# kcroker/Gadget-2.0.7-ngravs

Hardware: AMD Instinct MI355X
Metric: particle-steps/s (tree+PM) (higher is better)
Workload: dtype f64

## Files before the change

### gadget-2.0.7-ngravs_amd/__init__.py

```python
import ctypes as C
import os
import subprocess

import numpy as np

from . import abi, ic
from .abi import (Config, Particles, Stats, make_config, WALK_GROUP, WALK_STRICT,
                  LAW_NONE, LAW_NEWTON, LAW_NEG_NEWTON, LAW_YUKAWA, LAW_COLOYUK, LAW_BAMBAM, LAW_SOURCEBAM, LAW_TARGETBAM)

_HERE = os.path.dirname(os.path.abspath(__file__))
LIB_PATH = os.path.join(_HERE, "libngravs_hip.so")
_LIB = None

EXPORTS = [
    "ngravs_abi_version", "ngravs_build_info", "ngravs_config_default", "ngravs_create", "ngravs_destroy",
    "ngravs_set_fatal_handler", "ngravs_set_opening", "ngravs_set_walk_mode", "ngravs_set_softening", "ngravs_dd_record_bytes", "ngravs_get_config", "ngravs_set_tuning",
    "ngravs_memcpy", "ngravs_device_alloc", "ngravs_device_free",
    "ngravs_set_particles",
    "ngravs_set_old_acc", "ngravs_update_particles", "ngravs_force_update_tree", "ngravs_domain_decomposition", "ngravs_discard_grav_pm",
    "ngravs_force_treebuild", "ngravs_gravity_tree",
    "ngravs_pmforce_periodic", "ngravs_compute_accelerations", "ngravs_get_accel", "ngravs_get_stats", "ngravs_walk_unopened",
    "ngravs_get_domain", "ngravs_get_keys", "ngravs_get_order", "ngravs_get_shard", "ngravs_last_error",
    "ngravs_peano_hilbert_key", "ngravs_peano_keys", "ngravs_shortrange_table", "ngravs_direct_sum", "ngravs_direct_sum_targets",
    "ngravs_dd_num_local", "ngravs_dd_local_extent", "ngravs_dd_set_extent", "ngravs_get_domain_extent", "ngravs_dd_set_toptree",
    "ngravs_dd_get_toptree", "ngravs_dd_peano_order", "ngravs_dd_leaf_sums", "ngravs_dd_target_bounds", "ngravs_dd_keep_margin", "ngravs_dd_pack", "ngravs_dd_get_dest",
    "ngravs_dd_pack_leaves", "ngravs_dd_set_top", "ngravs_dd_recv_buffer", "ngravs_dd_apply_migration", "ngravs_dd_set_halo",
    "ngravs_dd_leaf_sums_kept", "ngravs_dd_pack_leaves_kept", "ngravs_dd_refresh_halo", "ngravs_dd_update_top", "ngravs_dd_get_kept",
    "ngravs_dd_set_ids", "ngravs_dd_get_ids",
    "ngravs_pm_slab_begin", "ngravs_pm_slab_pack", "ngravs_pm_slab_unpack", "ngravs_pm_slab_bytes",
]
HOST_EXPORTS = ["ngravs_host_comm_selftest", "ngravs_host_kept_step", "ngravs_host_toptree_borrow", "ngravs_host_domain_decomposition", "ngravs_host_domain_owners", "ngravs_host_domain_halo",
                "ngravs_host_plan_free", "ngravs_host_pmforce_periodic", "ngravs_host_compute_accelerations", "ngravs_host_split",
                "ngravs_host_pm_seconds", "ngravs_host_toptree_init", "ngravs_host_toptree_from_children", "ngravs_host_toptree_adapt",
                "ngravs_host_toptree_free", "ngravs_host_import_request", "ngravs_host_import_request_margin"]
RCCL_LIB_PATH = os.path.join(_HERE, "libngravs_rccl.so")
RCCL_EXPORTS = ["ngravs_rccl_selftest", "ngravs_rccl_unique_id", "ngravs_rccl_create", "ngravs_rccl_fill", "ngravs_rccl_destroy", "ngravs_rccl_stats",
                "ngravs_rccl_last_error", "ngravs_rccl_world", "ngravs_rccl_barrier", "ngravs_rccl_set_timeout"]


# ... 16 lines not shown
            raise NgravsError("libngravs_hip.so is not built (run __graft_entry__.build()); there is no CPU fallback")
        L = C.CDLL(LIB_PATH)
        L.ngravs_build_info.restype = C.c_char_p
        L.ngravs_last_error.restype = C.c_char_p
        L.ngravs_last_error.argtypes = [C.c_void_p]
        L.ngravs_peano_hilbert_key.restype = C.c_int64
        L.ngravs_peano_hilbert_key.argtypes = [C.c_int] * 4
        L.ngravs_force_treebuild.restype = C.c_int64
        L.ngravs_force_treebuild.argtypes = [C.c_void_p]
        for name in ("ngravs_destroy", "ngravs_domain_decomposition", "ngravs_gravity_tree",
                     "ngravs_pmforce_periodic", "ngravs_discard_grav_pm"):
            getattr(L, name).argtypes = [C.c_void_p]
        L.ngravs_compute_accelerations.argtypes = [C.c_void_p, C.c_int]
        L.ngravs_set_opening.argtypes = [C.c_void_p, C.c_double, C.c_double]
        L.ngravs_set_walk_mode.argtypes = [C.c_void_p, C.c_int]
        L.ngravs_set_softening.argtypes = [C.c_void_p, C.c_void_p]
        L.ngravs_dd_record_bytes.restype = C.c_int64
        L.ngravs_dd_record_bytes.argtypes = [C.c_void_p, C.c_int]
        L.ngravs_set_particles.argtypes = [C.c_void_p, C.c_void_p]
        L.ngravs_set_old_acc.argtypes = [C.c_void_p, C.c_void_p, C.c_int64, C.c_int]
        L.ngravs_get_accel.argtypes = [C.c_void_p, C.c_void_p, C.c_int64, C.c_void_p, C.c_int64, C.c_void_p, C.c_int64,
                                       C.c_void_p, C.c_int64, C.c_int, C.c_int]
        L.ngravs_set_tuning.argtypes = [C.c_void_p, C.c_char_p, C.c_double]
        L.ngravs_memcpy.argtypes = [C.c_void_p, C.c_void_p, C.c_void_p, C.c_int64, C.c_int]
        L.ngravs_get_stats.argtypes = [C.c_void_p, C.c_void_p]
        L.ngravs_get_domain.argtypes = [C.c_void_p, C.c_void_p]
        L.ngravs_get_keys.argtypes = [C.c_void_p, C.c_void_p, C.c_int]
        L.ngravs_get_order.argtypes = [C.c_void_p, C.c_void_p, C.c_int]
        L.ngravs_get_shard.argtypes = [C.c_void_p, C.c_void_p, C.c_void_p]
        L.ngravs_peano_keys.argtypes = [C.c_void_p, C.c_void_p, C.c_int64, C.c_void_p, C.c_double, C.c_int, C.c_void_p]
        L.ngravs_shortrange_table.argtypes = [C.c_void_p, C.c_void_p, C.c_void_p]
        L.ngravs_direct_sum.argtypes = [C.c_void_p, C.c_void_p, C.c_int64, C.c_void_p]
        L.ngravs_direct_sum_targets.argtypes = [C.c_void_p, C.c_void_p, C.c_void_p, C.c_void_p, C.c_int64, C.c_void_p]
        L.ngravs_dd_local_extent.argtypes = [C.c_void_p, C.c_void_p, C.c_void_p]
        L.ngravs_dd_set_extent.argtypes = [C.c_void_p, C.c_void_p, C.c_void_p]
        L.ngravs_get_config.argtypes = [C.c_void_p, C.c_void_p]
        L.ngravs_host_split.argtypes = [C.c_void_p, C.c_void_p, C.c_int64, C.c_int, C.c_double, C.c_void_p]
        L.ngravs_dd_pack.argtypes = [C.c_void_p, C.c_int, C.c_void_p, C.c_int, C.c_int, C.c_void_p, C.c_void_p, C.c_void_p]
        L.ngravs_host_toptree_init.argtypes = [C.c_void_p, C.c_int]
        L.ngravs_host_toptree_from_children.argtypes = [C.c_void_p, C.c_void_p, C.c_int32]
        L.ngravs_host_toptree_adapt.argtypes = [C.c_void_p, C.c_void_p, C.c_double, C.c_int, C.c_void_p]
        L.ngravs_host_toptree_free.argtypes = [C.c_void_p]
        L.ngravs_host_toptree_free.restype = None
        L.ngravs_host_import_request.argtypes = [C.c_void_p, C.c_void_p, C.c_void_p, C.c_void_p, C.c_void_p, C.c_int, C.c_void_p, C.c_void_p]
        L.ngravs_dd_apply_migration.argtypes = [C.c_void_p, C.c_void_p, C.c_int64]
        L.ngravs_dd_set_halo.argtypes = [C.c_void_p, C.c_void_p, C.c_int64]
# ... 241 lines not shown
```

### gadget-2.0.7-ngravs_amd/csrc/capi.hip

```cpp
#include "engine.hpp"
#include "../../include/ngravs_peano.h"
#include <chrono>
#include <cmath>

void ngravs_report(ngravs_ctx *ctx, int code, const std::string &msg)
{
  if(ctx)
    ctx->last_error = msg;
  if(ctx && ctx->on_fatal)
    ctx->on_fatal(code, msg.c_str());
  else
    fprintf(stderr, "task %d: endrun called with an error level of %d (%s)\n", ctx ? ctx->cfg.rank : 0, code, msg.c_str());
}

__global__ void k_pack_strided_f64(const unsigned char *src, long long stride, int ncomp, long long n, double *dst)
{
  long long i = blockIdx.x * (long long)blockDim.x + threadIdx.x;
  if(i >= n)
    return;
  const double *s = reinterpret_cast<const double *>(src + i * stride);
  for(int k = 0; k < ncomp; k++)
    dst[i * ncomp + k] = s[k];
}
__global__ void k_pack_type(const unsigned char *src, long long stride, long long n, int *dst, int *nbad)
// ... 409 lines not shown
    }
  else if(k == "walk_root")
    t.walk_root = iv != 0;
  else if(k == "walk_compact")
    t.walk_compact = iv != 0;
  else if(k == "walk_spread" && iv >= 0 && iv <= 64 && (iv & (iv - 1)) == 0)
    t.walk_spread = (int)iv;
  else if(k == "walk_sg" && iv >= 0 && iv <= 16)
    t.walk_sg = (int)iv;
  else if(k == "walk_ring" && iv >= 0 && iv <= 1)
    t.walk_ring = (int)iv;
  else if(k == "walk_ring_k" && iv >= 0 && iv <= 8)
    t.walk_ring_k = (int)iv;
  else if(k == "walk_nleaf" && iv >= -1 && iv <= 8)
    t.walk_nleaf = (int)iv;
  else if(k == "walk_exact_reach")
    t.walk_exact_reach = iv != 0;
  else if(k == "pm_notile")
    t.pm_notile = iv != 0;
  else if(k == "pm_fused_gather")
    t.pm_fused_gather = iv != 0;
  else if(k == "pm_tile_gather")
    t.pm_tile_gather = iv != 0;
  else if(k == "sort_full")
    t.sort_full = iv != 0;
  else if(k == "pm_tile8")
    t.pm_tile8 = iv != 0;
  else if(k == "tree_levelwise")
    t.tree_levelwise = iv != 0;
  else if(k == "dd_keep" && v >= 0 && v <= 0.25)
    t.dd_keep = v;
  else if(k == "moments_octet")
    t.moments_octet = iv != 0;
  else
    {
      ngravs_report(c, NGRAVS_ERR_ARG, "ngravs_set_tuning: unknown name or value out of range: " + k);
      return NGRAVS_ERR_ARG;
    }
  return NGRAVS_OK;
}

extern "C" int ngravs_memcpy(ngravs_ctx *c, void *dst, const void *src, int64_t bytes, int kind)
{
  if(!c || bytes < 0 || kind < 1 || kind > 3 || (bytes > 0 && (!dst || !src)))
    return NGRAVS_ERR_ARG;
  if(bytes == 0)
    return NGRAVS_OK;
  (void)hipSetDevice(c->cfg.device);
  HIP_TRY(c, hipStreamSynchronize(c->stream));
  HIP_TRY(c, hipMemcpy(dst, src, (size_t)bytes, kind == 1 ? hipMemcpyHostToDevice : (kind == 2 ? hipMemcpyDeviceToHost : hipMemcpyDeviceToDevice)));
  return NGRAVS_OK;
}

extern "C" int ngravs_device_alloc(ngravs_ctx *c, void **ptr, int64_t bytes)
{
  if(!c || !ptr || bytes < 0)
    return NGRAVS_ERR_ARG;
  *ptr = nullptr;
  (void)hipSetDevice(c->cfg.device);
  if(hipMalloc(ptr, (size_t)(bytes > 0 ? bytes : 1)) != hipSuccess)
    return NGRAVS_ERR_NOMEM;
// ... 1061 lines not shown
```

### gadget-2.0.7-ngravs_amd/csrc/engine.hpp

```cpp
#pragma once
#include <hip/hip_runtime.h>
#include <cstdint>
#include <cstdio>
#include <cstdlib>
#include <cstring>
#include <string>
#include <vector>
#include "../../include/ngravs_host.h"

#define NG_MAX NGRAVS_MAX_GRAVS
#define NTAB NGRAVS_NTAB
#define TREE_BITS NGRAVS_TREE_BITS
#define FLAG_BUCKET 64
#define FLAG_PSEUDO 128
#define FLAG_PARTIAL 256
#define MAX_LEVELS (TREE_BITS + 1)

struct ngravs_ctx;

#define HIP_TRY(ctx, expr)                                                                        \
  do                                                                                              \
    {                                                                                             \
      hipError_t e__ = (expr);                                                                    \
      if(e__ != hipSuccess)                                                                       \
// ... 57 lines not shown
  double ec[4];
  int src_in_box;
  int bam;
  int law_accel[NG_MAX][NG_MAX], law_spline[NG_MAX][NG_MAX];

};

struct TreeView
{
  const int *first, *count, *child, *flags;
  const int *npart;
  const double4 *geo, *mom;
  int nnodes;
  const int *ltab;
  int ltab_level;
  double ltab_corner[3], ltab_cl;
};

struct Tuning
{
  int walk_fused = 0, walk_waves = 0, walk_lcap = 0, walk_root = 0, walk_compact = 1, walk_spread = 0, walk_exact_reach = 0, walk_sg = 0, walk_nleaf = -1;
  long long walk_batch = 0;
  int pm_notile = 0, pm_fused_gather = 0, pm_tile_gather = 0, pm_tile8 = 0;
  int sort_full = 0;
  int tree_levelwise = 0;
  int moments_octet = 0;
  double dd_keep = 0;
  int walk_ring = 1;
  int walk_ring_k = 0;
};

#define TOP_CW(ng) (7 + 4 * (ng))
struct TopTree
{
  double total_count = 0;
  bool on = false;
  double import_reach = 0;
  ngravs_toptree h = {0, 0, 0, 0, nullptr, nullptr, nullptr, nullptr, nullptr};
  DevBuf<int> child, leaf;
  DevBuf<int> gcnt;
  DevBuf<unsigned char> info;
  DevBuf<double> gsum;
  DevBuf<int> leaf_owner;
  DevBuf<unsigned long long> reqmask;
  DevBuf<double> leaf_sums;
  DevBuf<int> own_leaf;
// ... 84 lines not shown
  DevBuf<int> d_levels;
  long long level_hint[MAX_LEVELS + 2] = {0};
  DevBuf<double> table;
  bool table_ready = false;
  DevBuf<double> lat;
  bool lat_ready = false;
  DevBuf<int> walk_stack;
  DevBuf<int> walk_tlist;
  DevBuf<unsigned char> walk_tmp;
  long long walk_ntargets = -1;
  bool walk_dense_tlist = false;
  int walk_spread = 0;
  int walk_sg = 1;
  long long walk_unopened = 0;
  int walk_unit_state = 4;
  double walk_ia_ratio = 0;
  bool all_active = true;
  DevBuf<int> walk_ovf;
  DevBuf<int> walk_counters;
  DevBuf<double> r_acc, r_pm, r_oldacc;
  DevBuf<int> r_nint;
  int pm_plan_n = 0;
  void *fft_fwd = nullptr, *fft_inv = nullptr;
  DevBuf<double> pm_rho;
  DevBuf<double> pm_force;
  DevBuf<double> pm_phi;
  DevBuf<double> pm_orig;
  DevBuf<double> out_tmp;
  DevBuf<float> out_tmpf;
  std::vector<unsigned char> host_stage;
  ngravs_stats_t stats;
  hipEvent_t ev0 = nullptr, ev1 = nullptr, evk0 = nullptr, evk1 = nullptr;
  std::vector<hipEvent_t> ev_batch;
  int walk_batches = 0;
  int walk_lcap = 0;
  int walk_scap = 0;
  std::string last_error;
};

int dom_find_extent(ngravs_ctx *c);
int dom_keys_and_sort(ngravs_ctx *c);
int dom_keys_only(ngravs_ctx *c, const double *d_pos, int64_t n, const double corner[3], double fac, int bits,
                  long long *d_keys);
int dd_local_extent(ngravs_ctx *c, double lo[3], double hi[3]);
void dd_apply_extent(ngravs_ctx *c, const double lo[3], const double hi[3]);
int dd_set_toptree(ngravs_ctx *c, int nnode, const int *child);
// ... 17 lines not shown
int tree_top_leaf_len(ngravs_ctx *c, double *dev_kept_sums, int stride);
int tree_top_refit(ngravs_ctx *c);
int dom_regather(ngravs_ctx *c);
static inline bool cfg_has_bam(const ngravs_config_t &cfg)
{
  for(int i = 0; i < cfg.n_gravs; i++)
    for(int j = 0; j < cfg.n_gravs; j++)
      if(cfg.law_accel[i][j] >= NGRAVS_LAW_BAMBAM || cfg.law_spline[i][j] >= NGRAVS_SPLINE_BAMBAM)
        return true;
  return false;
}
void make_walk_params(const ngravs_ctx *c, WalkParams *wp);
int walk_run(ngravs_ctx *c);
int walk_finish(ngravs_ctx *c);
int direct_run(ngravs_ctx *c, const int *d_idx, int64_t nt, double *d_acc);
int direct_run_targets(ngravs_ctx *c, const double4 *d_tpm, const int *d_ttype, int64_t nt, double *d_acc);
int eval_ring_slots(const WalkParams &wp, bool yuk, int waves);
int launch_eval_ring(ngravs_ctx *c, const TreeView &tv, const WalkParams &wp, bool yuk, int nblk, int waves, int K, const int *region,
                     const int *gcount, long long g0, long long nb, int lcap, int scap, int S, const int *tlist, int SG, long long t_count);
int pm_run(ngravs_ctx *c);
int pm_deposit(ngravs_ctx *c);
int pm_finish(ngravs_ctx *c);
void pm_release(ngravs_ctx *c);
int pmslab_begin(ngravs_ctx *c, int rank, int world, int bbox[6]);
int pmslab_pack(ngravs_ctx *c, int stage, const int *all_bbox, int64_t *send_counts, int64_t *recv_counts, void **send, void **recv);
int pmslab_unpack(ngravs_ctx *c, int stage);
void pmslab_release(ngravs_ctx *c);
void host_shortrange_table(const ngravs_config_t *cfg, double *force, double *pot);
double cfg_asmth(const ngravs_config_t *c);
double cfg_rcut(const ngravs_config_t *c);
```

### gadget-2.0.7-ngravs_amd/csrc/kernels_pm.hip

```cpp
#include "engine.hpp"
#include "pm_common.hpp"
#include <hipfft/hipfft.h>

__global__ void k_cic_deposit(const double4 *__restrict__ s_pm, const unsigned char *__restrict__ s_type,
                              const unsigned char *__restrict__ s_flag, long long n,
                              double to_slab, int N, int ng, const int *__restrict__ t2g_tab, double *__restrict__ rho)
{
  long long i = blockIdx.x * (long long)blockDim.x + threadIdx.x;
  if(i >= n || (s_flag[i] & 2))
    return;
  double4 p = s_pm[i];
  int g = t2g_tab[s_type[i]];
  const long long NZ = N + 2;
  double *grid = rho + (size_t)g * N * N * NZ;
  double dx, dy, dz;
  int sx = cell_of(p.x, to_slab, N, &dx), sy = cell_of(p.y, to_slab, N, &dy), sz = cell_of(p.z, to_slab, N, &dz);
  int sxx = sx + 1 == N ? 0 : sx + 1, syy = sy + 1 == N ? 0 : sy + 1, szz = sz + 1 == N ? 0 : sz + 1;
  double m = p.w;
  atomicAdd(&grid[((long long)sx * N + sy) * NZ + sz], m * (1.0 - dx) * (1.0 - dy) * (1.0 - dz));
  atomicAdd(&grid[((long long)sx * N + syy) * NZ + sz], m * (1.0 - dx) * dy * (1.0 - dz));
  atomicAdd(&grid[((long long)sx * N + sy) * NZ + szz], m * (1.0 - dx) * (1.0 - dy) * dz);
  atomicAdd(&grid[((long long)sx * N + syy) * NZ + szz], m * (1.0 - dx) * dy * dz);
  atomicAdd(&grid[((long long)sxx * N + sy) * NZ + sz], m * (dx) * (1.0 - dy) * (1.0 - dz));
  atomicAdd(&grid[((long long)sxx * N + syy) * NZ + sz], m * (dx)*dy * (1.0 - dz));
  atomicAdd(&grid[((long long)sxx * N + sy) * NZ + szz], m * (dx) * (1.0 - dy) * dz);
  atomicAdd(&grid[((long long)sxx * N + syy) * NZ + szz], m * (dx)*dy * dz);
}

template <int NG>
__global__ void k_green(const double2 *__restrict__ rho, double2 *__restrict__ phi, GreenParams gp)
{
  const int N = gp.N, NH = N / 2 + 1;
  long long idx = blockIdx.x * (long long)blockDim.x + threadIdx.x;
  long long total = (long long)N * N * NH;
  if(idx >= total)
    return;
  int z = (int)(idx % NH);
  int y = (int)((idx / NH) % N);
  int x = (int)(idx / ((long long)NH * N));
  double2 out[NG];
  green_mode<NG>(gp, x, y, z, rho, (size_t)total, (size_t)idx, out);
#pragma unroll
  for(int b = 0; b < NG; b++)
    phi[(size_t)b * total + idx] = out[b];
}

__global__ void k_gradient_gather(const double4 *__restrict__ s_pm, const unsigned char *__restrict__ s_type,
                                  const unsigned char *__restrict__ s_flag,
                                  long long first, long long n, double to_slab, int N, const int *__restrict__ t2g_tab,
                                  const double *__restrict__ phi, double fac, double *__restrict__ r_pm)
{
  long long i = blockIdx.x * (long long)blockDim.x + threadIdx.x;
  if(i >= n)
    return;
  i += first;
  if(s_flag[i] & 2)
    {
      r_pm[3 * i + 0] = r_pm[3 * i + 1] = r_pm[3 * i + 2] = 0.0;
      return;
    }
  double4 p = s_pm[i];
  int g = t2g_tab[s_type[i]];
  const long long NZ = N + 2;
  const double *grid = phi + (size_t)g * N * N * NZ;
  double dx, dy, dz;
  int sx = cell_of(p.x, to_slab, N, &dx), sy = cell_of(p.y, to_slab, N, &dy), sz = cell_of(p.z, to_slab, N, &dz);
  double wx[2] = {1.0 - dx, dx}, wy[2] = {1.0 - dy, dy}, wz[2] = {1.0 - dz, dz};
// ... 366 lines not shown
  r_pm[3 * i + 1] = acc[1];
  r_pm[3 * i + 2] = acc[2];
}

static int pm_tile_level(const ngravs_ctx *c, double to_slab, double max_cells = 16.0)
{
  if(!c->have_tree || c->tune.pm_notile)
    return -1;
  double len = c->dom[6];
  for(int l = 0; l < c->nlevels && l < TREE_BITS; l++, len *= 0.5)
    if(len * to_slab <= max_cells * 1.002)
      return (c->level_start[l + 1] - c->level_start[l] > 0) ? l : -1;
  return -1;
}

void pm_release(ngravs_ctx *c)
{
  if(c->fft_fwd)
    {
      hipfftDestroy(*(hipfftHandle *)c->fft_fwd);
      delete(hipfftHandle *)c->fft_fwd;
      c->fft_fwd = nullptr;
    }
  if(c->fft_inv)
    {
      hipfftDestroy(*(hipfftHandle *)c->fft_inv);
      delete(hipfftHandle *)c->fft_inv;
      c->fft_inv = nullptr;
    }
  c->pm_plan_n = 0;
}

int pm_deposit_tiles(ngravs_ctx *c, const MeshAddr &ma, double *dst)
{
  const int N = c->cfg.pmgrid, ng = c->cfg.n_gravs;
  const double to_slab = N / c->cfg.box_size;
  const int bs = 256;
  const bool t8 = c->tune.pm_tile8 != 0;
  const int tl = pm_tile_level(c, to_slab, t8 ? 8.0 : 16.0);
  if(tl < 0)
    return 1;
  const long long tl0 = c->level_start[tl], tln = c->level_start[tl + 1] - tl0;
  const int dt = t8 ? 10 : PM_DT;
  const size_t lds = sizeof(double) * ng * dt * dt * dt;
  auto launch_dep = [&](auto kern) -> int {
    HIP_TRY(c, hipFuncSetAttribute(reinterpret_cast<const void *>(kern), hipFuncAttributeMaxDynamicSharedMemorySize, (int)lds));
    hipLaunchKernelGGL(kern, dim3((unsigned)tln), dim3(t8 ? 256 : PM_TILE_THREADS), lds, c->stream, c->s_pm.p, c->s_type.p, c->s_active.p,
                       c->n_first.p, c->n_count.p, c->n_geo.p, (int)tl0, to_slab, N, c->d_counters.p + 8, dst, ma);
    return NGRAVS_OK;
  };
  int rc;
  if(t8)
// ... 11 lines not shown
}

int pm_deposit(ngravs_ctx *c)
{
  const int N = c->cfg.pmgrid, ng = c->cfg.n_gravs;
  const long long n = c->n;
  if(N <= 0 || !c->cfg.periodic)
    {
      ngravs_report(c, NGRAVS_ERR_ARG, "pmforce_periodic needs PERIODIC and PMGRID");
      return NGRAVS_ERR_ARG;
    }
  const size_t real_elems = (size_t)N * N * (N + 2);
  if(c->pm_rho.ensure(real_elems * ng) || c->pm_phi.ensure(real_elems * ng) || c->r_pm.ensure(3 * n) || c->d_counters.ensure(16))
    return NGRAVS_ERR_NOMEM;
  if(c->pm_plan_n != N)
    {
      pm_release(c);
      c->fft_fwd = new hipfftHandle;
      c->fft_inv = new hipfftHandle;
      FFT_TRY(c, hipfftPlan3d((hipfftHandle *)c->fft_fwd, N, N, N, HIPFFT_D2Z));
      FFT_TRY(c, hipfftPlan3d((hipfftHandle *)c->fft_inv, N, N, N, HIPFFT_Z2D));
      FFT_TRY(c, hipfftSetStream(*(hipfftHandle *)c->fft_fwd, c->stream));
      FFT_TRY(c, hipfftSetStream(*(hipfftHandle *)c->fft_inv, c->stream));
      c->pm_plan_n = N;
    }
  HIP_TRY(c, hipMemcpyAsync(c->d_counters.p + 8, c->cfg.type_to_grav, sizeof(int) * 6, hipMemcpyHostToDevice, c->stream));
  const double L = c->cfg.box_size, to_slab = N / L;
  HIP_TRY(c, hipMemsetAsync(c->pm_rho.p, 0, sizeof(double) * real_elems * ng, c->stream));
  const int bs = 256;
  unsigned nbp = (unsigned)((n + bs - 1) / bs);
  MeshAddr ma;
  ma.N = N;
  ma.brick = 0;
  for(int j = 0; j < 3; j++)
    {
      ma.lo[j] = 0;
      ma.ext[j] = N;
    }
  int rct = pm_deposit_tiles(c, ma, c->pm_rho.p);
  if(rct == 1)
    hipLaunchKernelGGL(k_cic_deposit, dim3(nbp), dim3(bs), 0, c->stream, c->s_pm.p, c->s_type.p, c->s_active.p, n, to_slab, N, ng,
                       c->d_counters.p + 8, c->pm_rho.p);
  else if(rct)
    return rct;
  HIP_TRY(c, hipGetLastError());
  return NGRAVS_OK;
}

int pm_finish(ngravs_ctx *c)
{
  const int N = c->cfg.pmgrid, ng = c->cfg.n_gravs;
  const long long n = c->n;
  const size_t real_elems = (size_t)N * N * (N + 2);
  const double L = c->cfg.box_size, to_slab = N / L;
  const int bs = 256;
  const int tl = pm_tile_level(c, to_slab);
  const long long tl0 = tl >= 0 ? c->level_start[tl] : 0, tln = tl >= 0 ? c->level_start[tl + 1] - tl0 : 0;
  (void)tln;
  for(int a = 0; a < ng; a++)
    FFT_TRY(c, hipfftExecD2Z(*(hipfftHandle *)c->fft_fwd, c->pm_rho.p + real_elems * a,
                             (hipfftDoubleComplex *)(c->pm_rho.p + real_elems * a)));
  GreenParams gp;
  make_green_params(c, &gp);
  long long modes = (long long)N * N * (N / 2 + 1);
  unsigned nbm = (unsigned)((modes + bs - 1) / bs);
  switch(ng)
    {
    case 1:
      hipLaunchKernelGGL(k_green<1>, dim3(nbm), dim3(bs), 0, c->stream, (const double2 *)c->pm_rho.p, (double2 *)c->pm_phi.p, gp);
      break;
    case 2:
      hipLaunchKernelGGL(k_green<2>, dim3(nbm), dim3(bs), 0, c->stream, (const double2 *)c->pm_rho.p, (double2 *)c->pm_phi.p, gp);
      break;
    default:
      hipLaunchKernelGGL(k_green<3>, dim3(nbm), dim3(bs), 0, c->stream, (const double2 *)c->pm_rho.p, (double2 *)c->pm_phi.p, gp);
      break;
    }
  for(int b = 0; b < ng; b++)
    FFT_TRY(c, hipfftExecZ2D(*(hipfftHandle *)c->fft_inv, (hipfftDoubleComplex *)(c->pm_phi.p + real_elems * b),
                             c->pm_phi.p + real_elems * b));
  double fac = c->cfg.G / (M_PI * L);
  fac *= 1 / (2 * L / N);
  if(c->cfg.world_size > 1)
    HIP_TRY(c, hipMemsetAsync(c->r_pm.p, 0, sizeof(double) * 3 * n, c->stream));
  unsigned nbg = (unsigned)((c->shard_count + bs - 1) / bs);
  const int gl = c->tune.pm_tile_gather ? pm_tile_level(c, to_slab, 8.0) : -1;
  if(gl >= 0)
    {
      const long long gl0 = c->level_start[gl], gln = c->level_start[gl + 1] - gl0;
      const size_t lds = sizeof(double) * ng * PM_G8 * PM_G8 * PM_G8;
      auto launch_gat = [&](auto kern) -> int {
        HIP_TRY(c, hipFuncSetAttribute(reinterpret_cast<const void *>(kern), hipFuncAttributeMaxDynamicSharedMemorySize, (int)lds));
        hipLaunchKernelGGL(kern, dim3((unsigned)gln), dim3(256), lds, c->stream, c->s_pm.p, c->s_type.p, c->s_active.p, c->n_first.p,
                           c->n_count.p, c->n_geo.p, (int)gl0, (long long)c->shard_first, (long long)c->shard_count, to_slab, N,
                           c->d_counters.p + 8, c->pm_phi.p, fac, c->r_pm.p);
        return NGRAVS_OK;
      };
      int rc = ng == 1 ? launch_gat(k_gradient_gather_tiled<1>) : (ng == 2 ? launch_gat(k_gradient_gather_tiled<2>) : launch_gat(k_gradient_gather_tiled<3>));
      if(rc)
        return rc;
      if(gl0 > 0)
        hipLaunchKernelGGL(k_gradient_gather_loose, dim3((unsigned)((8 * gl0 + bs - 1) / bs)), dim3(bs), 0, c->stream, c->s_pm.p,
                           c->s_type.p, c->s_active.p, c->n_child.p, (int)gl0, (long long)c->shard_first, (long long)c->shard_count,
// ... 47 lines not shown
```

### gadget-2.0.7-ngravs_amd/csrc/pm_common.hpp

```cpp
#pragma once
#include "engine.hpp"
#include <hipfft/hipfft.h>
#include <cmath>

__device__ __forceinline__ int cell_of(double x, double to_slab, int N, double *frac)
{
  int s = (int)(to_slab * x);
  if(s >= N)
    s = N - 1;
  *frac = to_slab * x - s;
  return s;
}

__device__ __forceinline__ int wrapN(int a, int N) { return a < 0 ? a + N : (a >= N ? a - N : a); }

struct MeshAddr
{
  int N, brick;
  int lo[3], ext[3];
  __device__ __forceinline__ long long cell(int x, int y, int z) const
  {
    if(brick)
      return ((long long)wrapN(wrapN(x, N) - lo[0], N) * ext[1] + wrapN(wrapN(y, N) - lo[1], N)) * ext[2] + wrapN(wrapN(z, N) - lo[2], N);
    return ((long long)wrapN(x, N) * N + wrapN(y, N)) * (N + 2) + wrapN(z, N);
  }
  __host__ __device__ long long species_stride() const
  {
    return brick ? (long long)ext[0] * ext[1] * ext[2] : (long long)N * N * (N + 2);
  }
};

struct GreenParams
{
  int ng, N;
  double asmth2;
  double ym2;
  double yfac;
  double cN[NG_MAX][NG_MAX], cY[NG_MAX][NG_MAX];
};


template <int NG>
__device__ __forceinline__ void green_mode(const GreenParams &gp, int x, int y, int z, const double2 *__restrict__ rho, size_t sstride,
                                           size_t idx, double2 (&out)[NG])
{
  const int N = gp.N;
  double kx = x > N / 2 ? x - N : x, ky = y > N / 2 ? y - N : y, kz = z;
  double k2 = kx * kx + ky * ky + kz * kz;
#pragma unroll
  for(int b = 0; b < NG; b++)
    out[b].x = out[b].y = 0;
  if(k2 > 0)
    {
      double fx = 1, fy = 1, fz = 1;
      if(kx != 0)
        {
          fx = (M_PI * kx) / N;
          fx = sin(fx) / fx;
        }
      if(ky != 0)
        {
          fy = (M_PI * ky) / N;
          fy = sin(fy) / fy;
        }
      if(kz != 0)
        {
          fz = (M_PI * kz) / N;
          fz = sin(fz) / fz;
        }
      double ff = 1 / (fx * fy * fz);
      double common = -exp(-k2 * gp.asmth2) * ff * ff * ff * ff;
      double gN = 1.0 / k2, gY = 1.0 / (k2 + gp.ym2) * gp.yfac;
#pragma unroll
      for(int a = 0; a < NG; a++)
        {
          double2 r = rho[(size_t)a * sstride + idx];
#pragma unroll
          for(int b = 0; b < NG; b++)
            {
              double smth = (gp.cN[a][b] * gN + gp.cY[a][b] * gY) * common;
              out[b].x += r.x * smth;
              out[b].y += r.y * smth;
            }
        }
    }
}

static inline void make_green_params(const ngravs_ctx *c, GreenParams *gpp)
{
  GreenParams &gp = *gpp;
  const int N = c->cfg.pmgrid, ng = c->cfg.n_gravs;
  const double L = c->cfg.box_size;
  memset(&gp, 0, sizeof(gp));
  gp.ng = ng;
  gp.N = N;
  gp.asmth2 = (2 * M_PI) * c->asmth / L;
  gp.asmth2 *= gp.asmth2;
  double ym = c->cfg.yukawa_imass / (2 * M_PI);
  gp.ym2 = ym * ym;
  gp.yfac = exp(-ym * ym * gp.asmth2);
  for(int a = 0; a < ng; a++)
    for(int b = 0; b < ng; b++)
      {
        int law = c->cfg.law_greens[a][b];
        gp.cN[a][b] = law == NGRAVS_LAW_NEWTON || law == NGRAVS_LAW_COLOYUK ? 1.0 : (law == NGRAVS_LAW_NEG_NEWTON ? -1.0 : 0.0);
        gp.cY[a][b] = law == NGRAVS_LAW_YUKAWA || law == NGRAVS_LAW_COLOYUK ? 1.0 : 0.0;
      }
}
// ... 15 lines not shown
```

### include/ngravs_hip.h

```cpp
#ifndef NGRAVS_HIP_H
#define NGRAVS_HIP_H

#include <stdint.h>
#include <stddef.h>

#ifdef __cplusplus
extern "C" {
#endif

#define NGRAVS_ABI_VERSION 3
#define NGRAVS_MAX_GRAVS 3
#define NGRAVS_NTYPES 6
#define NGRAVS_NTAB 2048
#define NGRAVS_ASMTH 1.25
#define NGRAVS_RCUT 4.5
#define NGRAVS_BITS_PER_DIMENSION 18
#define NGRAVS_GROUP_REACH 4.5
#define NGRAVS_TREE_BITS 21

typedef enum {
  NGRAVS_LAW_NONE = 0,
  NGRAVS_LAW_NEWTON = 1,
  NGRAVS_LAW_NEG_NEWTON = 2,
  NGRAVS_LAW_YUKAWA = 3,
// ... 75 lines not shown
typedef struct {
  int64_t n_active;
  int64_t n_nodes;
  double interactions;
  double t_domain, t_peano, t_treebuild, t_treewalk, t_pm;
  double walk_kernel_ms;
  double reserved[7];
} ngravs_stats_t;

typedef struct ngravs_ctx ngravs_ctx;
typedef void (*ngravs_fatal_fn)(int code, const char *msg);

int ngravs_abi_version(void);
const char *ngravs_build_info(void);
void ngravs_config_default(ngravs_config_t *cfg);
int ngravs_create(const ngravs_config_t *cfg, ngravs_ctx **out);
void ngravs_destroy(ngravs_ctx *ctx);
void ngravs_set_fatal_handler(ngravs_ctx *ctx, ngravs_fatal_fn fn);
int ngravs_set_opening(ngravs_ctx *ctx, double err_tol_theta, double err_tol_force_acc);
int ngravs_set_walk_mode(ngravs_ctx *ctx, int walk_mode);
int ngravs_set_softening(ngravs_ctx *ctx, const double force_softening[NGRAVS_NTYPES]);
int ngravs_get_config(ngravs_ctx *ctx, ngravs_config_t *out);
int ngravs_set_tuning(ngravs_ctx *ctx, const char *name, double value);
int ngravs_memcpy(ngravs_ctx *ctx, void *dst, const void *src, int64_t bytes, int kind);
int ngravs_device_alloc(ngravs_ctx *ctx, void **ptr, int64_t bytes);
int ngravs_device_free(ngravs_ctx *ctx, void *ptr);

int ngravs_set_particles(ngravs_ctx *ctx, const ngravs_particles_t *p);
int ngravs_update_particles(ngravs_ctx *ctx, const ngravs_particles_t *p);
int ngravs_set_old_acc(ngravs_ctx *ctx, const double *old_acc, int64_t stride, int on_device);

int ngravs_domain_decomposition(ngravs_ctx *ctx);
int ngravs_discard_grav_pm(ngravs_ctx *ctx);
int64_t ngravs_force_treebuild(ngravs_ctx *ctx);
int ngravs_force_update_tree(ngravs_ctx *ctx);
int ngravs_gravity_tree(ngravs_ctx *ctx);
int ngravs_pmforce_periodic(ngravs_ctx *ctx);
int ngravs_compute_accelerations(ngravs_ctx *ctx, int pm_step);

int ngravs_get_accel(ngravs_ctx *ctx, double *grav_accel, int64_t accel_stride,
                     double *grav_pm, int64_t pm_stride, double *old_acc, int64_t old_acc_stride,
                     float *grav_cost, int64_t cost_stride, int on_device, int only_active);
int ngravs_get_stats(ngravs_ctx *ctx, ngravs_stats_t *out);
int ngravs_walk_unopened(ngravs_ctx *ctx, int64_t *count);
int ngravs_get_domain(ngravs_ctx *ctx, double out[8]);
int ngravs_get_keys(ngravs_ctx *ctx, int64_t *keys, int on_device);
// ... 53 lines not shown
```

Before: 611.6 million.

## Fuse x-axis FFT, Green's function and inverse x-FFT into one LDS kernel

Replaces the full 3D forward FFT, the separate Green-function kernel and the full 3D inverse FFT with batched 2D (y,z) hipFFT transforms around a custom kernel. That kernel loads x-columns into LDS, runs a radix-8 forward FFT along x, applies the Green's function, runs the inverse x-FFT and writes phi back. This removes two full-grid memory passes (the x-axis FFT stages and the separate Green pass). It adds a hand-written FFT with precomputed twiddles, limited to power-of-two grids with 1-3 gravity types, and falls back to the old path otherwise.

```diff
diff --git a/gadget-2.0.7-ngravs_amd/__init__.py b/gadget-2.0.7-ngravs_amd/__init__.py
--- a/gadget-2.0.7-ngravs_amd/__init__.py
+++ b/gadget-2.0.7-ngravs_amd/__init__.py
@@ -14,7 +14,7 @@
 
 EXPORTS = [
     "ngravs_abi_version", "ngravs_build_info", "ngravs_config_default", "ngravs_create", "ngravs_destroy",
-    "ngravs_set_fatal_handler", "ngravs_set_opening", "ngravs_set_walk_mode", "ngravs_set_softening", "ngravs_dd_record_bytes", "ngravs_get_config", "ngravs_set_tuning",
+    "ngravs_set_fatal_handler", "ngravs_set_opening", "ngravs_set_walk_mode", "ngravs_set_softening", "ngravs_dd_record_bytes", "ngravs_get_config", "ngravs_set_tuning", "ngravs_pm_twiddles",
     "ngravs_memcpy", "ngravs_device_alloc", "ngravs_device_free",
     "ngravs_set_particles",
     "ngravs_set_old_acc", "ngravs_update_particles", "ngravs_force_update_tree", "ngravs_domain_decomposition", "ngravs_discard_grav_pm",
@@ -77,6 +77,7 @@
         L.ngravs_get_accel.argtypes = [C.c_void_p, C.c_void_p, C.c_int64, C.c_void_p, C.c_int64, C.c_void_p, C.c_int64,
                                        C.c_void_p, C.c_int64, C.c_int, C.c_int]
         L.ngravs_set_tuning.argtypes = [C.c_void_p, C.c_char_p, C.c_double]
+        L.ngravs_pm_twiddles.argtypes = [C.c_int, C.c_void_p]
         L.ngravs_memcpy.argtypes = [C.c_void_p, C.c_void_p, C.c_void_p, C.c_int64, C.c_int]
         L.ngravs_get_stats.argtypes = [C.c_void_p, C.c_void_p]
         L.ngravs_get_domain.argtypes = [C.c_void_p, C.c_void_p]
diff --git a/gadget-2.0.7-ngravs_amd/csrc/capi.hip b/gadget-2.0.7-ngravs_amd/csrc/capi.hip
--- a/gadget-2.0.7-ngravs_amd/csrc/capi.hip
+++ b/gadget-2.0.7-ngravs_amd/csrc/capi.hip
@@ -455,6 +455,8 @@
     t.pm_fused_gather = iv != 0;
   else if(k == "pm_tile_gather")
     t.pm_tile_gather = iv != 0;
+  else if(k == "pm_kspace_fused")
+    t.pm_kspace_fused = iv != 0;
   else if(k == "sort_full")
     t.sort_full = iv != 0;
   else if(k == "pm_tile8")
@@ -470,6 +472,14 @@
       ngravs_report(c, NGRAVS_ERR_ARG, "ngravs_set_tuning: unknown name or value out of range: " + k);
       return NGRAVS_ERR_ARG;
     }
+  return NGRAVS_OK;
+}
+
+extern "C" int ngravs_pm_twiddles(int n, double *out)
+{
+  if(n < 8 || n % 8 || !out)
+    return NGRAVS_ERR_ARG;
+  pm_twiddles(n, out);
   return NGRAVS_OK;
 }
 
diff --git a/gadget-2.0.7-ngravs_amd/csrc/engine.hpp b/gadget-2.0.7-ngravs_amd/csrc/engine.hpp
--- a/gadget-2.0.7-ngravs_amd/csrc/engine.hpp
+++ b/gadget-2.0.7-ngravs_amd/csrc/engine.hpp
@@ -103,6 +103,7 @@
   int walk_fused = 0, walk_waves = 0, walk_lcap = 0, walk_root = 0, walk_compact = 1, walk_spread = 0, walk_exact_reach = 0, walk_sg = 0, walk_nleaf = -1;
   long long walk_batch = 0;
   int pm_notile = 0, pm_fused_gather = 0, pm_tile_gather = 0, pm_tile8 = 0;
+  int pm_kspace_fused = 1;
   int sort_full = 0;
   int tree_levelwise = 0;
   int moments_octet = 0;
@@ -233,6 +234,8 @@
   DevBuf<int> r_nint;
   int pm_plan_n = 0;
   void *fft_fwd = nullptr, *fft_inv = nullptr;
+  void *fft2_fwd = nullptr, *fft2_inv = nullptr;
+  DevBuf<double> pm_tw;
   DevBuf<double> pm_rho;
   DevBuf<double> pm_force;
   DevBuf<double> pm_phi;
@@ -296,6 +299,7 @@
 int pm_deposit(ngravs_ctx *c);
 int pm_finish(ngravs_ctx *c);
 void pm_release(ngravs_ctx *c);
+void pm_twiddles(int N, double *out);
 int pmslab_begin(ngravs_ctx *c, int rank, int world, int bbox[6]);
 int pmslab_pack(ngravs_ctx *c, int stage, const int *all_bbox, int64_t *send_counts, int64_t *recv_counts, void **send, void **recv);
 int pmslab_unpack(ngravs_ctx *c, int stage);
diff --git a/gadget-2.0.7-ngravs_amd/csrc/kernels_pm.hip b/gadget-2.0.7-ngravs_amd/csrc/kernels_pm.hip
--- a/gadget-2.0.7-ngravs_amd/csrc/kernels_pm.hip
+++ b/gadget-2.0.7-ngravs_amd/csrc/kernels_pm.hip
@@ -1,6 +1,8 @@
 #include "engine.hpp"
 #include "pm_common.hpp"
 #include <hipfft/hipfft.h>
+#include <type_traits>
+#include <vector>
 
 __global__ void k_cic_deposit(const double4 *__restrict__ s_pm, const unsigned char *__restrict__ s_type,
                               const unsigned char *__restrict__ s_flag, long long n,
@@ -43,6 +45,223 @@
 #pragma unroll
   for(int b = 0; b < NG; b++)
     phi[(size_t)b * total + idx] = out[b];
+}
+
+#define KX_COL(N) ((N) + 2)
+
+__device__ __forceinline__ int kx_swz(int i) { return i ^ ((i >> 3) & 7); }
+__device__ __forceinline__ double2 cadd(double2 a, double2 b) { return make_double2(a.x + b.x, a.y + b.y); }
+__device__ __forceinline__ double2 csub(double2 a, double2 b) { return make_double2(a.x - b.x, a.y - b.y); }
+__device__ __forceinline__ double2 cmul(double2 a, double2 w) { return make_double2(a.x * w.x - a.y * w.y, a.x * w.y + a.y * w.x); }
+template <bool INV> __device__ __forceinline__ double2 mul_si(double2 a)
+{
+  return INV ? make_double2(-a.y, a.x) : make_double2(a.y, -a.x);
+}
+
+template <int R, bool INV> __device__ __forceinline__ void kx_dft(double2 (&v)[R])
+{
+  if constexpr(R == 2)
+    {
+      double2 t = v[0];
+      v[0] = cadd(t, v[1]);
+      v[1] = csub(t, v[1]);
+    }
+  else if constexpr(R == 4)
+    {
+      double2 t0 = cadd(v[0], v[2]), t1 = csub(v[0], v[2]), t2 = cadd(v[1], v[3]), t3 = mul_si<INV>(csub(v[1], v[3]));
+      v[0] = cadd(t0, t2);
+      v[2] = csub(t0, t2);
+      v[1] = cadd(t1, t3);
+      v[3] = csub(t1, t3);
+    }
+  else
+    {
+      double2 e[4] = {v[0], v[2], v[4], v[6]}, o[4] = {v[1], v[3], v[5], v[7]};
+      kx_dft<4, INV>(e);
+      kx_dft<4, INV>(o);
+      const double h = 0.70710678118654752440;
+      double2 s1 = mul_si<INV>(o[1]), s3 = mul_si<INV>(o[3]);
+      o[1] = make_double2(h * (o[1].x + s1.x), h * (o[1].y + s1.y));
+      o[2] = mul_si<INV>(o[2]);
+      o[3] = make_double2(h * (s3.x - o[3].x), h * (s3.y - o[3].y));
+#pragma unroll
+      for(int k = 0; k < 4; k++)
+        {
+          v[k] = cadd(e[k], o[k]);
+          v[k + 4] = csub(e[k], o[k]);
+        }
+    }
+}
+
+template <int N, int R, int NS, bool INV>
+__device__ __forceinline__ void kx_pass(double2 *col, int lane, const double2 *__restrict__ tw)
+{
+  constexpr int NB = N / R, K = (NB + 63) / 64;
+  double2 v[K][R];
+#pragma unroll
+  for(int k = 0; k < K; k++)
+    if(NB % 64 == 0 || lane + 64 * k < NB)
+#pragma unroll
+      for(int r = 0; r < R; r++)
+        v[k][r] = col[kx_swz(lane + 64 * k + r * NB)];
+  __builtin_amdgcn_wave_barrier();
+#pragma unroll
+  for(int k = 0; k < K; k++)
+    {
+      const int b = lane + 64 * k;
+      if(NB % 64 != 0 && b >= NB)
+        continue;
+      const int j = b & (NS - 1);
+      if(NS > 1)
+#pragma unroll
+        for(int r = 1; r < R; r++)
+          {
+            double2 w = tw[r * j * (N / (NS * R))];
+            if(!INV)
+              w.y = -w.y;
+            v[k][r] = cmul(v[k][r], w);
+          }
+      kx_dft<R, INV>(v[k]);
+      const int o = (b - j) * R + j;
+#pragma unroll
+      for(int r = 0; r < R; r++)
+        col[kx_swz(o + r * NS)] = v[k][r];
+    }
+  __builtin_amdgcn_wave_barrier();
+}
+
+template <int N, int NS, bool INV> __device__ __forceinline__ void kx_fft(double2 *col, int lane, const double2 *__restrict__ tw)
+{
+  if constexpr(NS < N)
+    {
+      constexpr int R = N / NS >= 8 ? 8 : N / NS;
+      kx_pass<N, R, NS, INV>(col, lane, tw);
+      kx_fft<N, NS * R, INV>(col, lane, tw);
+    }
+}
+
+constexpr size_t kx_lds_size(int NG, int N, int ZR) { return 16 * ((size_t)NG * ZR * KX_COL(N) + N) + 8 * (size_t)N; }
+
+template <int NG, int N, int ZR>
+__global__ __launch_bounds__(64 * ZR) void k_kspace_x(const double2 *__restrict__ rho, double2 *__restrict__ phi,
+                                                             const double2 *__restrict__ tw, GreenParams gp)
+{
+  constexpr int T = 64 * ZR;
+  extern __shared__ double2 kx_lds[];
+  constexpr int NH = N / 2 + 1, NZG = (NH + ZR - 1) / ZR, P = KX_COL(N);
+  constexpr size_t S = (size_t)N * N * NH;
+  constexpr int NE = NG * N * ZR, NPT = (NE + T - 1) / T;
+  constexpr int NBLK = N * NZG, TPX = NBLK / 8;
+  const int xcd = blockIdx.x & 7, per = gridDim.x >> 3;
+  const int tid = threadIdx.x, lane = tid & 63, wave = tid >> 6;
+  double2 *twl = kx_lds + NG * ZR * P;
+  double *sxl = (double *)(twl + N);
+  for(int t = tid; t < N; t += T)
+    {
+      twl[t] = tw[t];
+      sxl[t] = green_sinc(green_k(t, N), N);
+    }
+  static_assert(T % ZR == 0, "the Green phase keeps one z' per thread");
+  double2 pre[NPT];
+  auto fetch = [&](int k) {
+    const int l = xcd * TPX + k, y = l / NZG, z0 = (l % NZG) * ZR, nz = NH - z0 < ZR ? NH - z0 : ZR;
+#pragma unroll
+    for(int p = 0; p < NPT; p++)
+      {
+        const int i = tid + p * T, c = i % ZR, x = (i / ZR) % N, a = i / (ZR * N);
+        pre[p] = make_double2(0.0, 0.0);
+        if((NE % T == 0 || i < NE) && c < nz)
+          pre[p] = rho[a * S + ((size_t)x * N + y) * NH + z0 + c];
+      }
+  };
+  int k = blockIdx.x >> 3;
+  if(k < TPX)
+    fetch(k);
+  for(; k < TPX; k += per)
+    {
+      const int l = xcd * TPX + k, y = l / NZG, z0 = (l % NZG) * ZR, nz = NH - z0 < ZR ? NH - z0 : ZR;
+      __syncthreads();
+#pragma unroll
+      for(int p = 0; p < NPT; p++)
+        {
+          const int i = tid + p * T, c = i % ZR, x = (i / ZR) % N, a = i / (ZR * N);
+          if(NE % T == 0 || i < NE)
+            kx_lds[(a * ZR + c) * P + kx_swz(x)] = pre[p];
+        }
+      __syncthreads();
+      if(k + per < TPX)
+        fetch(k + per);
+      for(int col = wave; col < NG * ZR; col += T / 64)
+        if(col % ZR < nz)
+          kx_fft<N, 1, false>(kx_lds + col * P, lane, twl);
+      __syncthreads();
+      {
+        const int c = tid % ZR;
+        const double ky = green_k(y, N), kz = z0 + c, fy = green_sinc(ky, N), fz = green_sinc(kz, N);
+        if(c < nz)
+          for(int x = tid / ZR; x < N; x += T / ZR)
+            {
+              double2 out[NG];
+              green_mode_f<NG>(gp, green_k(x, N), ky, kz, sxl[x], fy, fz, kx_lds, (size_t)ZR * P, (size_t)c * P + kx_swz(x), out);
+#pragma unroll
+              for(int b = 0; b < NG; b++)
+                kx_lds[(b * ZR + c) * P + kx_swz(x)] = out[b];
+            }
+      }
+      __syncthreads();
+      for(int col = wave; col < NG * ZR; col += T / 64)
+        if(col % ZR < nz)
+          kx_fft<N, 1, true>(kx_lds + col * P, lane, twl);
+      __syncthreads();
+#pragma unroll
+      for(int p = 0; p < NPT; p++)
+        {
+          const int i = tid + p * T, c = i % ZR, x = (i / ZR) % N, b = i / (ZR * N);
+          if((NE % T == 0 || i < NE) && c < nz)
+            phi[b * S + ((size_t)x * N + y) * NH + z0 + c] = kx_lds[(b * ZR + c) * P + kx_swz(x)];
+        }
+    }
+}
+
+static int kx_zr(int N, int ng)
+{
+  if(N <= 512 && kx_lds_size(ng, N, 8) <= (size_t)160 * 1024)
+    return 8;
+  return kx_lds_size(ng, N, 4) <= (size_t)160 * 1024 ? 4 : 0;
+}
+
+static int kx_log2n(int N, int ng)
+{
+  int l = 0;
+  while((1 << l) < N)
+    l++;
+  if((1 << l) != N || l < 5 || l > 10 || ng < 1 || ng > 3)
+    return 0;
+  return kx_zr(N, ng) ? l : 0;
+}
+
+void pm_twiddles(int N, double *out)
+{
+  const long double pi = 3.141592653589793238462643383279502884L;
+  const int q = N / 4;
+  for(int t = 0; t < N; t++)
+    {
+      const int k = t / q, r = t % q;
+      double c, s;
+      if(2 * r <= q)
+        {
+          c = (double)cosl(2 * pi * r / N);
+          s = (double)sinl(2 * pi * r / N);
+        }
+      else
+        {
+          c = (double)sinl(2 * pi * (q - r) / N);
+          s = (double)cosl(2 * pi * (q - r) / N);
+        }
+      const double cc[4] = {c, -s, -c, s}, ss[4] = {s, c, -s, -c};
+      out[2 * t] = cc[k];
+      out[2 * t + 1] = ss[k];
+    }
 }
 
 __global__ void k_gradient_gather(const double4 *__restrict__ s_pm, const unsigned char *__restrict__ s_type,
@@ -455,12 +674,13 @@
       delete(hipfftHandle *)c->fft_fwd;
       c->fft_fwd = nullptr;
     }
-  if(c->fft_inv)
-    {
-      hipfftDestroy(*(hipfftHandle *)c->fft_inv);
-      delete(hipfftHandle *)c->fft_inv;
-      c->fft_inv = nullptr;
-    }
+  for(void **h : {&c->fft_inv, &c->fft2_fwd, &c->fft2_inv})
+    if(*h)
+      {
+        hipfftDestroy(*(hipfftHandle *)*h);
+        delete(hipfftHandle *)*h;
+        *h = nullptr;
+      }
   c->pm_plan_n = 0;
 }
 
@@ -518,6 +738,22 @@
       FFT_TRY(c, hipfftPlan3d((hipfftHandle *)c->fft_inv, N, N, N, HIPFFT_Z2D));
       FFT_TRY(c, hipfftSetStream(*(hipfftHandle *)c->fft_fwd, c->stream));
       FFT_TRY(c, hipfftSetStream(*(hipfftHandle *)c->fft_inv, c->stream));
+      if(kx_log2n(N, ng))
+        {
+          int n2[2] = {N, N}, rembed[2] = {N, N + 2}, cembed[2] = {N, N / 2 + 1};
+          const int rdist = N * (N + 2), cdist = N * (N / 2 + 1);
+          c->fft2_fwd = new hipfftHandle;
+          c->fft2_inv = new hipfftHandle;
+          FFT_TRY(c, hipfftPlanMany((hipfftHandle *)c->fft2_fwd, 2, n2, rembed, 1, rdist, cembed, 1, cdist, HIPFFT_D2Z, N));
+          FFT_TRY(c, hipfftPlanMany((hipfftHandle *)c->fft2_inv, 2, n2, cembed, 1, cdist, rembed, 1, rdist, HIPFFT_Z2D, N));
+          FFT_TRY(c, hipfftSetStream(*(hipfftHandle *)c->fft2_fwd, c->stream));
+          FFT_TRY(c, hipfftSetStream(*(hipfftHandle *)c->fft2_inv, c->stream));
+          std::vector<double> tw(2 * (size_t)N);
+          pm_twiddles(N, tw.data());
+          if(c->pm_tw.ensure(2 * (size_t)N))
+            return NGRAVS_ERR_NOMEM;
+          HIP_TRY(c, hipMemcpy(c->pm_tw.p, tw.data(), sizeof(double) * 2 * N, hipMemcpyHostToDevice));
+        }
       c->pm_plan_n = N;
     }
   HIP_TRY(c, hipMemcpyAsync(c->d_counters.p + 8, c->cfg.type_to_grav, sizeof(int) * 6, hipMemcpyHostToDevice, c->stream));
@@ -543,6 +779,52 @@
   return NGRAVS_OK;
 }
 
+static int launch_kspace_x(ngravs_ctx *c, int l, const GreenParams &gp)
+{
+  const int N = 1 << l, ng = gp.ng, zr = kx_zr(N, ng);
+  const size_t lds = kx_lds_size(ng, N, zr);
+  const int ntile = N * ((N / 2 + 1 + zr - 1) / zr);
+  int ncu = 256;
+  hipDeviceProp_t prop;
+  if(hipGetDeviceProperties(&prop, c->cfg.device) == hipSuccess && prop.multiProcessorCount > 0)
+    ncu = prop.multiProcessorCount;
+  auto go = [&](auto kern) -> int {
+    HIP_TRY(c, hipFuncSetAttribute(reinterpret_cast<const void *>(kern), hipFuncAttributeMaxDynamicSharedMemorySize, (int)lds));
+    int per_cu = 1;
+    HIP_TRY(c, hipOccupancyMaxActiveBlocksPerMultiprocessor(&per_cu, kern, 64 * zr, lds));
+    int g = ncu * (per_cu > 0 ? per_cu : 1);
+    g = g < ntile ? g : ntile;
+    const unsigned nblk = (unsigned)(g >= 8 ? g & ~7 : 8);
+    hipLaunchKernelGGL(kern, dim3(nblk), dim3(64 * zr), lds, c->stream, (const double2 *)c->pm_rho.p, (double2 *)c->pm_phi.p,
+                       (const double2 *)c->pm_tw.p, gp);
+    return NGRAVS_OK;
+  };
+  auto by_n = [&](auto ngc) -> int {
+    constexpr int G = decltype(ngc)::value;
+    switch(l)
+      {
+      case 5: return go(k_kspace_x<G, 32, 8>);
+      case 6: return go(k_kspace_x<G, 64, 8>);
+      case 7: return go(k_kspace_x<G, 128, 8>);
+      case 8: return go(k_kspace_x<G, 256, 8>);
+      case 9:
+        if constexpr(G < 3)
+          return go(k_kspace_x<G, 512, 8>);
+        else
+          return go(k_kspace_x<G, 512, 4>);
+      default:
+        if constexpr(G < 3)
+          return go(k_kspace_x<G, 1024, 4>);
+        return NGRAVS_ERR_ARG;
+      }
+  };
+  int rc = ng == 1 ? by_n(std::integral_constant<int, 1>()) : (ng == 2 ? by_n(std::integral_constant<int, 2>()) : by_n(std::integral_constant<int, 3>()));
+  if(rc)
+    return rc;
+  HIP_TRY(c, hipGetLastError());
+  return NGRAVS_OK;
+}
+
 int pm_finish(ngravs_ctx *c)
 {
   const int N = c->cfg.pmgrid, ng = c->cfg.n_gravs;
@@ -553,28 +835,44 @@
   const int tl = pm_tile_level(c, to_slab);
   const long long tl0 = tl >= 0 ? c->level_start[tl] : 0, tln = tl >= 0 ? c->level_start[tl + 1] - tl0 : 0;
   (void)tln;
-  for(int a = 0; a < ng; a++)
-    FFT_TRY(c, hipfftExecD2Z(*(hipfftHandle *)c->fft_fwd, c->pm_rho.p + real_elems * a,
-                             (hipfftDoubleComplex *)(c->pm_rho.p + real_elems * a)));
   GreenParams gp;
   make_green_params(c, &gp);
-  long long modes = (long long)N * N * (N / 2 + 1);
-  unsigned nbm = (unsigned)((modes + bs - 1) / bs);
-  switch(ng)
-    {
-    case 1:
-      hipLaunchKernelGGL(k_green<1>, dim3(nbm), dim3(bs), 0, c->stream, (const double2 *)c->pm_rho.p, (double2 *)c->pm_phi.p, gp);
-      break;
-    case 2:
-      hipLaunchKernelGGL(k_green<2>, dim3(nbm), dim3(bs), 0, c->stream, (const double2 *)c->pm_rho.p, (double2 *)c->pm_phi.p, gp);
-      break;
-    default:
-      hipLaunchKernelGGL(k_green<3>, dim3(nbm), dim3(bs), 0, c->stream, (const double2 *)c->pm_rho.p, (double2 *)c->pm_phi.p, gp);
-      break;
-    }
-  for(int b = 0; b < ng; b++)
-    FFT_TRY(c, hipfftExecZ2D(*(hipfftHandle *)c->fft_inv, (hipfftDoubleComplex *)(c->pm_phi.p + real_elems * b),
-                             c->pm_phi.p + real_elems * b));
+  const int kxl = c->tune.pm_kspace_fused && c->fft2_fwd ? kx_log2n(N, ng) : 0;
+  if(kxl)
+    {
+      for(int a = 0; a < ng; a++)
+        FFT_TRY(c, hipfftExecD2Z(*(hipfftHandle *)c->fft2_fwd, c->pm_rho.p + real_elems * a,
+                                 (hipfftDoubleComplex *)(c->pm_rho.p + real_elems * a)));
+      int rc = launch_kspace_x(c, kxl, gp);
+      if(rc)
+        return rc;
+      for(int b = 0; b < ng; b++)
+        FFT_TRY(c, hipfftExecZ2D(*(hipfftHandle *)c->fft2_inv, (hipfftDoubleComplex *)(c->pm_phi.p + real_elems * b),
+                                 c->pm_phi.p + real_elems * b));
+    }
+  else
+    {
+      for(int a = 0; a < ng; a++)
+        FFT_TRY(c, hipfftExecD2Z(*(hipfftHandle *)c->fft_fwd, c->pm_rho.p + real_elems * a,
+                                 (hipfftDoubleComplex *)(c->pm_rho.p + real_elems * a)));
+      long long modes = (long long)N * N * (N / 2 + 1);
+      unsigned nbm = (unsigned)((modes + bs - 1) / bs);
+      switch(ng)
+        {
+        case 1:
+          hipLaunchKernelGGL(k_green<1>, dim3(nbm), dim3(bs), 0, c->stream, (const double2 *)c->pm_rho.p, (double2 *)c->pm_phi.p, gp);
+          break;
+        case 2:
+          hipLaunchKernelGGL(k_green<2>, dim3(nbm), dim3(bs), 0, c->stream, (const double2 *)c->pm_rho.p, (double2 *)c->pm_phi.p, gp);
+          break;
+        default:
+          hipLaunchKernelGGL(k_green<3>, dim3(nbm), dim3(bs), 0, c->stream, (const double2 *)c->pm_rho.p, (double2 *)c->pm_phi.p, gp);
+          break;
+        }
+      for(int b = 0; b < ng; b++)
+        FFT_TRY(c, hipfftExecZ2D(*(hipfftHandle *)c->fft_inv, (hipfftDoubleComplex *)(c->pm_phi.p + real_elems * b),
+                                 c->pm_phi.p + real_elems * b));
+    }
   double fac = c->cfg.G / (M_PI * L);
   fac *= 1 / (2 * L / N);
   if(c->cfg.world_size > 1)
diff --git a/gadget-2.0.7-ngravs_amd/csrc/pm_common.hpp b/gadget-2.0.7-ngravs_amd/csrc/pm_common.hpp
--- a/gadget-2.0.7-ngravs_amd/csrc/pm_common.hpp
+++ b/gadget-2.0.7-ngravs_amd/csrc/pm_common.hpp
@@ -40,34 +40,29 @@
 };
 
 
+__device__ __forceinline__ double green_k(int x, int N) { return x > N / 2 ? x - N : x; }
+
+__device__ __forceinline__ double green_sinc(double k, int N)
+{
+  double f = 1;
+  if(k != 0)
+    {
+      f = (M_PI * k) / N;
+      f = sin(f) / f;
+    }
+  return f;
+}
+
 template <int NG>
-__device__ __forceinline__ void green_mode(const GreenParams &gp, int x, int y, int z, const double2 *__restrict__ rho, size_t sstride,
-                                           size_t idx, double2 (&out)[NG])
+__device__ __forceinline__ void green_mode_f(const GreenParams &gp, double kx, double ky, double kz, double fx, double fy, double fz,
+                                             const double2 *__restrict__ rho, size_t sstride, size_t idx, double2 (&out)[NG])
 {
-  const int N = gp.N;
-  double kx = x > N / 2 ? x - N : x, ky = y > N / 2 ? y - N : y, kz = z;
   double k2 = kx * kx + ky * ky + kz * kz;
 #pragma unroll
   for(int b = 0; b < NG; b++)
     out[b].x = out[b].y = 0;
   if(k2 > 0)
     {
-      double fx = 1, fy = 1, fz = 1;
-      if(kx != 0)
-        {
-          fx = (M_PI * kx) / N;
-          fx = sin(fx) / fx;
-        }
-      if(ky != 0)
-        {
-          fy = (M_PI * ky) / N;
-          fy = sin(fy) / fy;
-        }
-      if(kz != 0)
-        {
-          fz = (M_PI * kz) / N;
-          fz = sin(fz) / fz;
-        }
       double ff = 1 / (fx * fy * fz);
       double common = -exp(-k2 * gp.asmth2) * ff * ff * ff * ff;
       double gN = 1.0 / k2, gY = 1.0 / (k2 + gp.ym2) * gp.yfac;
@@ -84,6 +79,15 @@
             }
         }
     }
+}
+
+template <int NG>
+__device__ __forceinline__ void green_mode(const GreenParams &gp, int x, int y, int z, const double2 *__restrict__ rho, size_t sstride,
+                                           size_t idx, double2 (&out)[NG])
+{
+  const int N = gp.N;
+  const double kx = green_k(x, N), ky = green_k(y, N), kz = z;
+  green_mode_f<NG>(gp, kx, ky, kz, green_sinc(kx, N), green_sinc(ky, N), green_sinc(kz, N), rho, sstride, idx, out);
 }
 
 static inline void make_green_params(const ngravs_ctx *c, GreenParams *gpp)
diff --git a/include/ngravs_hip.h b/include/ngravs_hip.h
--- a/include/ngravs_hip.h
+++ b/include/ngravs_hip.h
@@ -121,6 +121,7 @@
 int ngravs_set_softening(ngravs_ctx *ctx, const double force_softening[NGRAVS_NTYPES]);
 int ngravs_get_config(ngravs_ctx *ctx, ngravs_config_t *out);
 int ngravs_set_tuning(ngravs_ctx *ctx, const char *name, double value);
+int ngravs_pm_twiddles(int n, double *out);
 int ngravs_memcpy(ngravs_ctx *ctx, void *dst, const void *src, int64_t bytes, int kind);
 int ngravs_device_alloc(ngravs_ctx *ctx, void **ptr, int64_t bytes);
 int ngravs_device_free(ngravs_ctx *ctx, void *ptr);
```

Measured after the change: 624.6 million, median of 6. 1.02x the previous value.
